# nowal/MASt3R-SLAM

Hardware: AMD Instinct MI355X
Metric: keyframe-pair GN iters/sec @512×384, 256 edges; ATE-RMSE vs ref (higher is better)
Workload: dtype f32; 1 GPU; cfg3: gauss_newton_calib op call, 256 keyframe-pair edges (512 directed), 128 keyframes, 384x512, 10 GN iters/step, delta_thresh=0; edges=256, directed_edges=512, keyframes=128, H=384, W=512, parallelism=edge-sharded x1

## Files before the change

include/m3s_backend.h:

```cpp
#ifndef M3S_BACKEND_H
#define M3S_BACKEND_H

#include <stddef.h>
#include <stdint.h>

#ifdef __cplusplus
extern "C" {
#endif

enum {
    M3S_OK = 0,
    M3S_ERR_INVALID = 1,
    M3S_ERR_HIP = 2,
    M3S_ERR_WORKSPACE = 3,
    M3S_ERR_COMM = 4,
    M3S_ERR_TIMEOUT = 5
};

const char* m3s_last_error(void);
const char* m3s_version(void);
void m3s_shutdown(void);

enum {
    M3S_CONTRACT_NVCC = 0,
// ... 4 lines not shown

int m3s_iter_proj(const float* rays, const float* pts, const float* p_init,
                  float* p_new, uint8_t* converged,
                  int64_t B, int64_t H, int64_t W, int64_t N,
                  int max_iter, float lambda_init, float cost_thresh, void* stream);
int m3s_iter_proj_ex(const float* rays, const float* pts, const float* p_init,
                     float* p_new, uint8_t* converged,
                     int64_t B, int64_t H, int64_t W, int64_t N,
                     int max_iter, float lambda_init, float cost_thresh, int contract, void* stream);

int m3s_refine_matches_f16(const uint16_t* D11, const uint16_t* D21,
                           const int64_t* p1, int64_t* p1_new,
                           int64_t B, int64_t H, int64_t W, int64_t N, int64_t F,
                           int radius, int dilation_max, void* stream);
int m3s_refine_matches_f32(const float* D11, const float* D21,
                           const int64_t* p1, int64_t* p1_new,
                           int64_t B, int64_t H, int64_t W, int64_t N, int64_t F,
                           int radius, int dilation_max, void* stream);
int m3s_refine_matches_f64(const double* D11, const double* D21,
                           const int64_t* p1, int64_t* p1_new,
                           int64_t B, int64_t H, int64_t W, int64_t N, int64_t F,
                           int radius, int dilation_max, void* stream);

size_t m3s_match_workspace_bytes(int64_t B, int64_t H, int64_t W, int64_t F);
int m3s_match_iterative_proj(const float* X11, const float* X21, const float* D11, const float* D21,
                             const int64_t* idx_init, int64_t B, int64_t H, int64_t W, int64_t F,
                             int max_iter, float lambda_init, float cost_thresh, float dist_thresh,
                             int radius, int dilation_max, int contract, int64_t* idx_out,
                             uint8_t* valid_out, void* ws, size_t ws_bytes, void* stream);



void m3s_gn_debug_flags(int* out4);
void m3s_gn_pcg_stats(int* out5);
void m3s_gn_pcg_plan(int* out5);

int m3s_gn_check(void* stream);

enum { M3S_GN_POINTS = 0, M3S_GN_RAYS = 1, M3S_GN_CALIB = 2 };

typedef struct m3s_gn_args {
    int mode;
    float* Twc;
    const float* Xs;
    const float* Cs;
    const int64_t* ii;
    const int64_t* jj;
    const int64_t* idx;
    const uint8_t* valid;
    const float* Q;
    int64_t N, HW, E_total, E_local, edge_offset;
    float sigma0;
    float sigma1;
    float C_thresh, Q_thresh;
    const float* K;
    int height, width, pixel_border;
    float z_eps;
    int max_iter;
    float delta_thresh;
    float* dx;
    void* ws;
    size_t ws_bytes;
    void* comm;
    void* stream;
    int order;
    const int64_t* idx_b;
// ... 128 lines not shown
```

mast3r-slam_amd/csrc/gn_accum.hip:

```cpp
#include <hip/hip_runtime.h>

#include <algorithm>
#include <climits>
#include <cstdint>

#include "edge_reduce.h"
#include "gn_kernels.h"
#include "sim3.h"
#include "wave_reduce.h"

#ifndef M3S_ACC_SCHED_BARRIER
#define M3S_ACC_SCHED_BARRIER 0
#endif
#ifndef M3S_ACC_DIAG
#define M3S_ACC_DIAG 0
#endif

namespace m3s {

template <typename V>
struct VMask {
    typedef bool type;
};

// ... 278 lines not shown
}

__device__ __forceinline__ void block_partial(const float* accs, float* __restrict__ out, bool coh = false) {
    __shared__ float red[kAccThreads / 64][kNaccPad];
    const int tid = threadIdx.x, lane = tid & 63, wave = tid >> 6;
    static_assert(kNaccPad == 36, "reduce-scatter is laid out for 36 values");
    float w[18], x[9];
#pragma unroll
    for (int j = 0; j < 18; j++) w[j] = halfsum32(accs[j], j + 18 < kNacc ? accs[j + 18] : 0.0f);
#pragma unroll
    for (int j = 0; j < 9; j++) x[j] = row_sum16(halfsum16(w[j], w[j + 9]));
    if ((lane & 15) == 0) {
        const int r = lane >> 4;
#pragma unroll
        for (int j = 0; j < 9; j++) red[wave][j + 9 * r] = x[j];
    }
    __syncthreads();
    if (tid < kNacc) {
        float s = red[0][tid];
#pragma unroll
        for (int w = 1; w < kAccThreads / 64; w++) s += red[w][tid];
        if (coh)
            __hip_atomic_store(out + tid, s, __ATOMIC_RELAXED, __HIP_MEMORY_SCOPE_AGENT);
        else
            out[tid] = s;
    }
}


#ifndef M3S_RC_FACTOR
#define M3S_RC_FACTOR 1
#endif

template <int MODE, bool RC = false, bool PK = true, int NP = 4>
struct AccStage {
    static_assert(NP == 4 || NP == 2, "4 or 2 points per step");
    int cd[NP], sb[NP];
    __device__ __forceinline__ void set(int4 a, int4 b) {
        cd[0] = a.x; sb[0] = a.y; cd[1] = a.z; sb[1] = a.w;
        if constexpr (NP == 4) {
            cd[2] = b.x; sb[2] = b.y; cd[3] = b.z; sb[3] = b.w;
        }
    }
    float xv[3 * NP];
    float g[NP][3];
    const float* rc_tu = nullptr;
    const float* rc_tv = nullptr;
    unsigned rc_m = 0;
    int rc_sh = 0, rc_w = 1;
    int width = 1;

    template <int M>
    __device__ __forceinline__ void load(const float* __restrict__ Xj_b, const float* __restrict__ Xi_b,
                                         const float* __restrict__ Zi_b, int k) {
        if constexpr (RC) {
            const unsigned q = (unsigned)(((uint64_t)(unsigned)k * rc_m) >> rc_sh);
            const int u = k - (int)q * rc_w;
            if constexpr (NP == 4) {
                const float4 za = *reinterpret_cast<const float4*>(Xj_b + k);
                const float4 ta = *reinterpret_cast<const float4*>(rc_tu + u);
                const float t[8] = {za.x, za.y, za.z, za.w, ta.x, ta.y, ta.z, ta.w};
#pragma unroll
                for (int i = 0; i < 8; i++) xv[i] = t[i];
            } else {
                const float2 za = *reinterpret_cast<const float2*>(Xj_b + k);
                const float2 ta = *reinterpret_cast<const float2*>(rc_tu + u);
                xv[0] = za.x; xv[1] = za.y; xv[2] = ta.x; xv[3] = ta.y;
            }
            xv[2 * NP] = rc_tv[q];
        } else if constexpr (NP == 4) {
            const float4 a = *reinterpret_cast<const float4*>(Xj_b + (int64_t)k * 3);
            const float4 b = *reinterpret_cast<const float4*>(Xj_b + (int64_t)k * 3 + 4);
            const float4 c = *reinterpret_cast<const float4*>(Xj_b + (int64_t)k * 3 + 8);
            const float t[12] = {a.x, a.y, a.z, a.w, b.x, b.y, b.z, b.w, c.x, c.y, c.z, c.w};
#pragma unroll
            for (int i = 0; i < 12; i++) xv[i] = t[i];
        } else {
            const float2 a = *reinterpret_cast<const float2*>(Xj_b + (int64_t)k * 3);
            const float2 b = *reinterpret_cast<const float2*>(Xj_b + (int64_t)k * 3 + 2);
            const float2 c = *reinterpret_cast<const float2*>(Xj_b + (int64_t)k * 3 + 4);
            const float t[6] = {a.x, a.y, b.x, b.y, c.x, c.y};
#pragma unroll
            for (int i = 0; i < 6; i++) xv[i] = t[i];
        }
        int ind[NP];
#pragma unroll
        for (int s = 0; s < NP; s++) ind[s] = (M == GN_CALIB && PK) ? uv_index(cd[s], width) : (cd[s] & 0x7fffffff);
#pragma unroll
        for (int s = 0; s < NP; s++) {
            if constexpr (M == GN_CALIB) {
                if constexpr (PK)
                    g[s][2] = Zi_b[ind[s]];
                else
                    g[s][2] = Xi_b[(int64_t)ind[s] * 3 + 2];
            } else {
                const float* xp = Xi_b + (int64_t)ind[s] * 3;
                g[s][0] = xp[0];
                g[s][1] = xp[1];
                g[s][2] = xp[2];
            }
        }
    }

    template <int M>
    __device__ __forceinline__ void compute(const RelXf& T, const AccParams& P, float* __restrict__ acc) const {
        const int* codes = cd;
        const int* sqb = sb;
        float xj[3 * NP];
        constexpr bool kFactor = RC && M == GN_CALIB && M3S_RC_FACTOR;
        float Xr[3 * NP];
        if constexpr (kFactor) {
            const float tv = xv[2 * NP];
            const float B0 = fmaf(T.m[1], tv, T.m[2]), B1 = fmaf(T.m[4], tv, T.m[5]), B2 = fmaf(T.m[7], tv, T.m[8]);
#pragma unroll
            for (int s = 0; s < NP; s++) {
                const float z = xv[s], tu = xv[NP + s];
                Xr[3 * s] = fmaf(z, fmaf(T.m[0], tu, B0), T.t[0]);
                Xr[3 * s + 1] = fmaf(z, fmaf(T.m[3], tu, B1), T.t[1]);
                Xr[3 * s + 2] = fmaf(z, fmaf(T.m[6], tu, B2), T.t[2]);
            }
        } else if constexpr (RC) {
#pragma unroll
            for (int s = 0; s < NP; s++) {
                xj[3 * s] = xv[s] * xv[NP + s];
                xj[3 * s + 1] = xv[s] * xv[2 * NP];
                xj[3 * s + 2] = xv[s];
            }
        } else {
#pragma unroll
            for (int q = 0; q < 3 * NP; q++) xj[q] = xv[q];
        }
#pragma unroll
// ... 376 lines not shown
                const int ind = match_index(ids[s], vm[s], P.HW);
                const bool ok = vm[s] && (qs[s] > P.Q_thresh) && (raw.ci_all || raw.Ci_b[ind] > P.C_thresh) &&
                                (raw.cj_all || cjs[s] > P.C_thresh);
                code[s] = pack_code(ind, ok, P);
                sqb[s] = __float_as_int(sqrt_cr(qs[s]));
            }
            a = int4{code[0], sqb[0], code[1], sqb[1]};
            raw.pk_w[kk / 2] = a;
        } else if constexpr (FIRST) {
            const uchar4 vm4 = *reinterpret_cast<const uchar4*>(raw.valid + kk);
            const longlong2 id01 = *reinterpret_cast<const longlong2*>(raw.idx + kk);
            const longlong2 id23 = *reinterpret_cast<const longlong2*>(raw.idx + kk + 2);
            const float4 q4 = *reinterpret_cast<const float4*>(raw.Q + kk);
            const float4 cj4 =
                raw.cj_all ? make_float4(0.f, 0.f, 0.f, 0.f) : *reinterpret_cast<const float4*>(raw.Cj_b + kk);
            const bool vm[4] = {vm4.x != 0, vm4.y != 0, vm4.z != 0, vm4.w != 0};
            const int64_t ids[4] = {id01.x, id01.y, id23.x, id23.y};
            const float qs[4] = {q4.x, q4.y, q4.z, q4.w};
            const float cjs[4] = {cj4.x, cj4.y, cj4.z, cj4.w};
            int code[4], sqb[4];
#pragma unroll
            for (int s = 0; s < 4; s++) {
                const int ind = match_index(ids[s], vm[s], P.HW);
                const bool ok = vm[s] && (qs[s] > P.Q_thresh) && (raw.ci_all || raw.Ci_b[ind] > P.C_thresh) &&
                                (raw.cj_all || cjs[s] > P.C_thresh);
                code[s] = pack_code(ind, ok, P);
                sqb[s] = __float_as_int(sqrt_cr(qs[s]));
            }
            a = int4{code[0], sqb[0], code[1], sqb[1]};
            b = int4{code[2], sqb[2], code[3], sqb[3]};
            raw.pk_w[kk / 2] = a;
            raw.pk_w[kk / 2 + 1] = b;
        } else {
            a = pk_b[kk / 2];
            if constexpr (NP == 4) b = pk_b[kk / 2 + 1];
        }
    };
    int4 na = int4{0, 0, 0, 0}, nb = int4{0, 0, 0, 0};
    int k = k0 + NP * threadIdx.x;
    if (k < k1) records(k, na, nb);
    for (; k < k1; k += S) {
#if M3S_ACC_DIAG == 1
        if (k == k0 + NP * (int)threadIdx.x) {
            cur.set(na, nb);
            cur.template load<MODE>(Xj_b, Xi_b, Zi_b, k);
        }
        cur.template compute<MODE>(T, P, acc);
        __builtin_amdgcn_sched_barrier(0);
        continue;
#elif M3S_ACC_DIAG == 2
        cur.set(na, nb);
        if (k + S < k1) records(k + S, na, nb);
        cur.template load<MODE>(Xj_b, Xi_b, Zi_b, k);
        if (k == k0 + NP * (int)threadIdx.x) {
            cur.template compute<MODE>(T, P, acc);
        } else {
#pragma unroll
            for (int q = 0; q < 3 * NP; q++) asm volatile("" ::"v"(cur.xv[q]));
#pragma unroll
            for (int q = 0; q < NP; q++) asm volatile("" ::"v"(cur.g[q][2]), "v"(cur.g[q][0]), "v"(cur.cd[q]), "v"(cur.sb[q]));
        }
        continue;
#endif
        cur.set(na, nb);
        if (k + S < k1) records(k + S, na, nb);
        cur.template load<MODE>(Xj_b, Xi_b, Zi_b, k);
        cur.template compute<MODE>(T, P, acc);
    }
}


#ifndef M3S_ACC_WAVES
#define M3S_ACC_WAVES 1
#endif
#ifndef M3S_ACC_WAVES_RAYS
#define M3S_ACC_WAVES_RAYS M3S_ACC_WAVES
#endif
template <int MODE, bool FIRST>
constexpr int acc_waves() {
    return (MODE == GN_RAYS && !FIRST) ? M3S_ACC_WAVES_RAYS : M3S_ACC_WAVES;
}
struct FirstSrc {
    EdgeSrc es;
    const float* Cs;
    const int* cok;
    int4* pack_w;
};

template <int MODE, bool COMPACT, bool RCOK = false, bool FIRST = false>
__global__ __launch_bounds__(kAccThreads) __attribute__((amdgpu_waves_per_eu(acc_waves<MODE, FIRST>())))
void gn_accum_packed_kernel(
    const float* __restrict__ Twc, const float* __restrict__ Xs, const float* __restrict__ Zs,
    const int* __restrict__ ii_loc, const int* __restrict__ jj_loc, const int4* __restrict__ pack,
    AccParams P, const int4* __restrict__ sched, float* __restrict__ partials,
    const int* __restrict__ flags, const float* __restrict__ px, const int* __restrict__ pcnt,
    int* __restrict__ ecnt, double* __restrict__ edgeblk, FirstSrc fs) {
    const int4 tk = sched[blockIdx.x];
    if (flags[kFlagDone]) return;
    const int e = tk.x, c = tk.y, ix = tk.z, jx = tk.w;
    const RelXf T = rel_xf(rel_sim3(load_sim3(Twc + (int64_t)ix * 8), load_sim3(Twc + (int64_t)jx * 8)));

    const int HW = P.HW;
    const int64_t ebase = (int64_t)e * HW;
    const float* __restrict__ Xi_b = Xs + (int64_t)ix * HW * 3;
    const float* __restrict__ Zi_b = MODE == GN_CALIB ? inv_depths(Zs, P) + (int64_t)ix * HW : nullptr;
    const float* __restrict__ Xj_b = Xs + (int64_t)jx * HW * 3;
    const int4* __restrict__ pk_b = pack + ebase / 2;
    const int k0 = c * P.chunk;
    const int k1 = min(k0 + P.chunk, HW);

    float acc[kNacc];
#pragma unroll
    for (int q = 0; q < kNacc; q++) acc[q] = 0.0f;
    if constexpr (COMPACT) {
        const int64_t cb = ((int64_t)e * P.nchunks + c) * P.chunk;
        accum_steps<MODE, false, acc_np<MODE>()>(px + cb * 3, Xi_b, Zi_b, pack + cb / 2, 0, pcnt[(int64_t)e * P.nchunks + c], T, P,
                                 Zs, acc);
    } else if constexpr (FIRST) {
        RawSrc raw;
        fs.es.at(e, HW, raw.idx, raw.valid, raw.Q);
        raw.Ci_b = fs.Cs + (int64_t)ix * HW;
        raw.Cj_b = fs.Cs + (int64_t)jx * HW;
        raw.pk_w = fs.pack_w + ebase / 2;
        raw.ci_all = fs.cok != nullptr && fs.cok[ix] != 0;
        raw.cj_all = fs.cok != nullptr && fs.cok[jx] != 0;
        if (RCOK && flags[kFlagNotRay] == 0 && (P.width & 3) == 0)
            accum_steps<MODE, true, 4, true>(Zs + (int64_t)jx * HW, Xi_b, Zi_b, pk_b, k0, k1, T, P, Zs, acc, raw);
        else
            accum_steps<MODE, false, acc_np<MODE>(), true>(Xj_b, Xi_b, Zi_b, pk_b, k0, k1, T, P, Zs, acc, raw);
    } else if (RCOK && MODE == GN_CALIB && flags[kFlagNotRay] == 0 && (P.width & 3) == 0)
        accum_steps<MODE, true, acc_np<MODE>()>(Zs + (int64_t)jx * HW, Xi_b, Zi_b, pk_b, k0, k1, T, P, Zs, acc);
    else
        accum_steps<MODE, false, acc_np<MODE>()>(Xj_b, Xi_b, Zi_b, pk_b, k0, k1, T, P, Zs, acc);
    block_partial(acc, partials + ((int64_t)e * P.nchunks + c) * kNaccPad, ecnt != nullptr);
    if (ecnt != nullptr) {
        __shared__ int s_last;
        asm volatile("s_waitcnt vmcnt(0)" ::: "memory");
        __syncthreads();
        if (threadIdx.x == 0)
            s_last = __hip_atomic_fetch_add(ecnt + e, 1, __ATOMIC_RELAXED, __HIP_MEMORY_SCOPE_AGENT) == P.nchunks - 1;
        __syncthreads();
        if (s_last) {
            edge_reduce_body<true>(partials, P.nchunks, Twc, ii_loc, edgeblk, e);
            if (threadIdx.x == 0) __hip_atomic_store(ecnt + e, 0, __ATOMIC_RELAXED, __HIP_MEMORY_SCOPE_AGENT);
        }
    }
}

hipError_t launch_accum(int mode, bool vec, dim3 grid, hipStream_t st, const float* Twc,
                        const float* Xs, const float* Cs, const int* ii_loc, const int* jj_loc,
                        const EdgeSrc& es, const AccParams& P, const int4* sched, float* partials,
                        const int* flags) {
#define M3S_ACC(MODE, V)                                                                    \
    hipLaunchKernelGGL((gn_accum_kernel<MODE, V>), grid, dim3(kAccThreads), 0, st, Twc, Xs, \
                       Cs, ii_loc, jj_loc, es, P, sched, partials, flags)
    if (mode == GN_RAYS) {
        if (vec) M3S_ACC(GN_RAYS, true); else M3S_ACC(GN_RAYS, false);
    } else if (mode == GN_CALIB) {
        if (vec) M3S_ACC(GN_CALIB, true); else M3S_ACC(GN_CALIB, false);
    } else {
        if (vec) M3S_ACC(GN_POINTS, true); else M3S_ACC(GN_POINTS, false);
    }
#undef M3S_ACC
    return hipGetLastError();
}

hipError_t launch_pack_pre(hipStream_t st, const float* Xs, int64_t N, const float* Cs, const AccParams& P, int* cok,
                           float* Zs, int* flags, const float* K) {
    if (cok != nullptr && N > 0) {
        const int bx = (int)std::max<int64_t>(1, std::min<int64_t>((P.HW + 1023) / 1024, 8192 / std::max<int64_t>(N, 1)));
        hipLaunchKernelGGL(gn_cpass_kernel, dim3(bx, (unsigned)N), dim3(256), 0, st, Cs, P, cok, flags);
    }
    if (Zs) {
        const int64_t total = N * (int64_t)P.HW;
        const int bx = (int)std::max<int64_t>(std::min<int64_t>((P.HW + 255) / 256,
                                                                std::max<int64_t>(8192 / std::max<int64_t>(N, 1), 2)),
                                              (std::max(P.width, P.height) + 255) / 256);
        hipLaunchKernelGGL(gn_depth_kernel, dim3(bx, (unsigned)N), dim3(256), 0, st, Xs, total, Zs, P, flags, K);
    }
    return hipGetLastError();
}

hipError_t launch_pack(int mode, hipStream_t st, int E_local, const float* Xs, int64_t N, const float* Cs,
                       const int* ii_loc, const int* jj_loc, const EdgeSrc& es, const AccParams& P, int* cok,
                       int4* pack, float* px, int* pcnt, const int* flags, bool skip_pack) {
    if (E_local > 0 && px) {
        const dim3 grid((unsigned)P.nchunks, (unsigned)E_local);
        int2* pk = reinterpret_cast<int2*>(pack);
        if (mode == GN_RAYS)
            hipLaunchKernelGGL(gn_pack_compact_kernel<GN_RAYS>, grid, dim3(kAccThreads), 0, st, Xs, Cs, ii_loc,
                               jj_loc, es, P, pk, px, pcnt, flags);
        else if (mode == GN_CALIB)
            hipLaunchKernelGGL(gn_pack_compact_kernel<GN_CALIB>, grid, dim3(kAccThreads), 0, st, Xs, Cs, ii_loc,
                               jj_loc, es, P, pk, px, pcnt, flags);
        else
            hipLaunchKernelGGL(gn_pack_compact_kernel<GN_POINTS>, grid, dim3(kAccThreads), 0, st, Xs, Cs, ii_loc,
                               jj_loc, es, P, pk, px, pcnt, flags);
    } else if (E_local > 0) {
        const dim3 grid((unsigned)((P.HW / 4 + kAccThreads - 1) / kAccThreads), (unsigned)E_local);
        if (!skip_pack)
            hipLaunchKernelGGL(gn_pack_kernel, grid, dim3(kAccThreads), 0, st, Cs, ii_loc, jj_loc, es,
                               P, cok, pack, flags);
    }
    return hipGetLastError();
}

hipError_t launch_accum_packed(int mode, dim3 grid, hipStream_t st, const float* Twc,
                               const float* Xs, const float* Zs, const int* ii_loc,
                               const int* jj_loc, const int4* pack, const AccParams& P,
                               const int4* sched, float* partials, const int* flags, const float* px,
                               const int* pcnt, int* ecnt, double* edgeblk, const EdgeSrc* first_es,
                               const float* Cs, const int* cok) {
    if (first_es != nullptr) {
        if (px != nullptr) return hipErrorInvalidValue;
        const FirstSrc fs{*first_es, Cs, cok, const_cast<int4*>(pack)};
        if (mode == GN_RAYS)
            hipLaunchKernelGGL((gn_accum_packed_kernel<GN_RAYS, false, false, true>), grid, dim3(kAccThreads), 0, st,
                               Twc, Xs, Zs, ii_loc, jj_loc, pack, P, sched, partials, flags, px, pcnt, ecnt,
                               edgeblk, fs);
        else if (mode == GN_POINTS)
            hipLaunchKernelGGL((gn_accum_packed_kernel<GN_POINTS, false, false, true>), grid, dim3(kAccThreads), 0, st,
                               Twc, Xs, Zs, ii_loc, jj_loc, pack, P, sched, partials, flags, px, pcnt, ecnt,
                               edgeblk, fs);
        else if (P.raycheck)
            hipLaunchKernelGGL((gn_accum_packed_kernel<GN_CALIB, false, true, true>), grid, dim3(kAccThreads), 0, st,
                               Twc, Xs, Zs, ii_loc, jj_loc, pack, P, sched, partials, flags, px, pcnt, ecnt,
                               edgeblk, fs);
        else
            hipLaunchKernelGGL((gn_accum_packed_kernel<GN_CALIB, false, false, true>), grid, dim3(kAccThreads), 0, st,
                               Twc, Xs, Zs, ii_loc, jj_loc, pack, P, sched, partials, flags, px, pcnt, ecnt,
                               edgeblk, fs);
        return hipGetLastError();
    }
    const FirstSrc fs0{};
#define M3S_ACCP(MODE, CP, RC)                                                                       \
    hipLaunchKernelGGL((gn_accum_packed_kernel<MODE, CP, RC>), grid, dim3(kAccThreads), 0, st, Twc, Xs, Zs, \
                       ii_loc, jj_loc, pack, P, sched, partials, flags, px, pcnt, ecnt, edgeblk, fs0)
#define M3S_ACCP2(MODE, CP) M3S_ACCP(MODE, CP, false)
    const bool cp = px != nullptr;
    if (mode == GN_RAYS) {
        if (cp) M3S_ACCP2(GN_RAYS, true); else M3S_ACCP2(GN_RAYS, false);
    } else if (mode == GN_CALIB) {
        if (cp) M3S_ACCP2(GN_CALIB, true);
        else if (P.raycheck) M3S_ACCP(GN_CALIB, false, true);
        else M3S_ACCP2(GN_CALIB, false);
    } else {
        if (cp) M3S_ACCP2(GN_POINTS, true); else M3S_ACCP2(GN_POINTS, false);
    }
#undef M3S_ACCP2
#undef M3S_ACCP
    return hipGetLastError();
}

}
```

mast3r-slam_amd/csrc/gn_driver.hip:

```cpp
#include <hip/hip_runtime.h>

#include <algorithm>
#include <chrono>
#include <cstdlib>
#include <cstdarg>
#include <cstdio>
#include <cstring>
#include <functional>
#include <map>
#include <mutex>
#include <set>
#include <string>
#include <utility>
#include <vector>

#include "../../include/m3s_backend.h"
#include "gn_kernels.h"
#include "m3s_common.h"
#include "m3s_comm.h"
#include "sparse_plan.h"

namespace m3s {

namespace {
// ... 6 lines not shown
    std::vector<hipEvent_t> pool;
    std::vector<hipEvent_t> marks;
    hipEvent_t get() {
        if (pool.empty()) {
            static const bool sysfence = env_int("M3S_PROF_SYSFENCE", 0) != 0;
            hipEvent_t e;
            if (sysfence || hipEventCreateWithFlags(&e, hipEventDisableSystemFence) != hipSuccess) {
                (void)hipGetLastError();
                if (hipEventCreate(&e) != hipSuccess) return nullptr;
            }
            return e;
        }
        hipEvent_t e = pool.back();
        pool.pop_back();
        return e;
    }
    bool accum_only = false;
    std::vector<char> first;
    void mark(hipStream_t st, bool accum = false, bool first_pack = false) {
        if (!on || (accum_only && !accum)) return;
        hipEvent_t e = get();
        if (e && hipEventRecord(e, st) == hipSuccess) {
            marks.push_back(e);
            if (accum_only && marks.size() % 2 == 0) first.push_back(first_pack);
        }
    }
};
Prof g_prof;
std::vector<double> g_prof_launch_ms;
std::vector<double> g_prof_solve_ms;
}

int g_dbg_flags[4] = {0, 0, 0, 0};
int g_dbg_pcg[5] = {0, 0, 0, 0, 0};
int g_dbg_pcg_plan[5] = {0, 0, 0, 0, 0};

void set_error(const char* fmt, ...) {
    char buf[1024];
    va_list ap;
    va_start(ap, fmt);
    vsnprintf(buf, sizeof(buf), fmt, ap);
    va_end(ap);
    g_err = buf;
}

const char* get_error() { return g_err.c_str(); }

namespace {
struct HostResources {
    std::mutex mu;
    std::vector<std::pair<void*, void (*)(void*)>> items;
    bool shut = false;
};
HostResources& host_resources() {
    static HostResources* r = new HostResources;
    return *r;
}
}

void register_host_resource(void* obj, void (*release)(void*)) {
    HostResources& r = host_resources();
    std::lock_guard<std::mutex> lk(r.mu);
    r.items.emplace_back(obj, release);
}

namespace {
// ... 580 lines not shown
                "gauss_newton_calib: K / image size required");
    M3S_REQUIRE(a.Twc && a.Xs && a.Cs && a.dx, "gauss_newton: null pointer");
    if (a.E_total > 0) M3S_REQUIRE(a.ii && a.jj, "gauss_newton: null ii/jj");
    if (a.E_local > 0) M3S_REQUIRE(a.idx && a.valid && a.Q, "gauss_newton: null edge data");
    if (a.idx_b || a.valid_b || a.Q_b) {
        M3S_REQUIRE(a.idx_b && a.valid_b && a.Q_b, "gauss_newton: incomplete second edge half");
        M3S_REQUIRE(a.E_a >= 0 && a.E_a <= a.E_local, "gauss_newton: bad edge split E_a = %lld",
                    (long long)a.E_a);
    }
    const size_t need = make_layout(a.mode, a.N, a.HW, a.E_total, a.E_local).total;
    M3S_REQUIRE(a.ws != nullptr && a.ws_bytes >= need,
                "gauss_newton: workspace too small (%zu < %zu bytes)", a.ws_bytes, need);
    return M3S_OK;
}

Plan& tls_plan() {
    static thread_local Plan p;
    return p;
}
SparsePlan& tls_sparse_plan() {
    static thread_local SparsePlan sp;
    return sp;
}

struct Ctx {
    bool need_slotmap = false;
    bool packed = false;
    bool compact = false;
    bool ref_order = false;
    bool pack_issued = false;
    bool acc_enqueued = false;
    bool gathered = false;
    bool first_pack = false;
    RefParams R;
    Layout L;
    Plan& plan = tls_plan();
    SparsePlan& sp = tls_sparse_plan();
    AccParams P;
    EdgeSrc es{};
    bool vec;
    char* ws;
    hipStream_t st = nullptr;
    char* dyn = nullptr;
    size_t o_dense = 0, o_linv = 0, o_slot = 0;
    double* eall = nullptr;
    double* eblk() const {
        return eall ? eall + (size_t)plan.grank * plan.gchunk * kEdgeBlk : at<double>(L.edgeblk);
    }
    const double* eblk_all() const { return eall ? eall : at<double>(L.edgeblk); }
    int chol_epoch = 0;
    int pcg_launches = 0;
    bool inv_pending = false;
    hipEvent_t inv_done = nullptr;
    bool may_timeout = false;
    template <typename T>
    T* at(size_t off) const { return reinterpret_cast<T*>(ws + off); }
    template <typename T>
    T* dyn_at(size_t off) const { return reinterpret_cast<T*>(dyn + off); }
    int alloc_dense(int npad, int npose) {
        size_t off = 0;
        auto take = [&](size_t bytes) {
            size_t o = off;
            off = align_up(off + std::max<size_t>(bytes, 8), 256);
            return o;
        };
        o_dense = take(sizeof(double) * (size_t)(npad + kCholTile) * npad);
// ... 44 lines not shown
    const auto s0 = std::chrono::steady_clock::now();
    const Layout& L = c.L;
    AccParams& P = c.P;
    P.s0_inv = 1.0f / a.sigma0;
    P.s1_inv = (a.mode == M3S_GN_POINTS) ? 0.0f : 1.0f / a.sigma1;
    P.C_thresh = a.C_thresh;
    P.Q_thresh = a.Q_thresh;
    P.pb_lo = (float)a.pixel_border;
    P.pb_hi_u = (float)(a.width - 1 - a.pixel_border);
    P.pb_hi_v = (float)(a.height - 1 - a.pixel_border);
    P.z_eps = a.z_eps;
    P.width = a.width > 0 ? a.width : 1;
    P.height = a.height;
    {
        int l = 0;
        while ((1LL << l) < P.width) l++;
        const unsigned long long num = 1ULL << (31 + l);
        P.div_m = (unsigned)((num + (unsigned long long)P.width - 1) / (unsigned long long)P.width);
        P.div_sh = 31 + l;
    }
    P.HW = (int)a.HW;
    P.chunk = chunk_points(a.HW, L.nchunks);
    P.nchunks = L.nchunks;
    P.nkf = (int)a.N;
    auto al16 = [](const void* ptr) { return ((uintptr_t)ptr & 15) == 0; };
    const bool two = a.idx_b != nullptr;
    c.es.idx[0] = a.idx;
    c.es.valid[0] = a.valid;
    c.es.Q[0] = a.Q;
    c.es.idx[1] = two ? a.idx_b : a.idx;
    c.es.valid[1] = two ? a.valid_b : a.valid;
    c.es.Q[1] = two ? a.Q_b : a.Q;
    c.es.E_a = two ? (int)a.E_a : (int)a.E_local;
    c.vec = (a.HW % 4 == 0) && al16(a.Xs) && al16(a.Cs) && al16(a.idx) && al16(a.valid) &&
            al16(a.Q) && (!two || (al16(a.idx_b) && al16(a.valid_b) && al16(a.Q_b)));
    const int pack_mode = env_int("M3S_GN_PACK", 1);
    c.packed = c.vec && a.E_local > 0 && (pack_mode == 2 || (pack_mode == 1 && a.max_iter >= 3));
    c.compact = c.packed && env_int("M3S_GN_COMPACT", 0) != 0;
    if (a.mode == M3S_GN_CALIB && (a.width >= 65536 || a.height >= 32768)) c.packed = c.compact = false;
    P.pack_uv = c.packed && a.mode == M3S_GN_CALIB;
    P.raycheck = c.packed && !c.compact && a.mode == M3S_GN_CALIB && env_int("M3S_GN_RAYCHECK", 1) != 0;

    c.ref_order = gn_order(a) == M3S_GN_ORDER_REFERENCE;
    if (c.ref_order) {
        c.packed = false;
        RefParams& R = c.R;
        R.s0_inv = (float)(1.0 / (double)a.sigma0);
        R.s1_inv = (a.mode == M3S_GN_POINTS) ? 0.0f : (float)(1.0 / (double)a.sigma1);
        R.C_thresh = a.C_thresh;
        R.Q_thresh = a.Q_thresh;
        R.z_eps = a.z_eps;
        R.width = a.width > 0 ? a.width : 1;
        R.height = a.height;
        R.pixel_border = a.pixel_border;
        R.HW = a.HW;
        R.variant = env_int("M3S_GN_REF_VARIANT", 0);
        R.contract = a.contract;
    }
    int* dflags = c.at<int>(L.flags);
    int* dcok = c.at<int>(L.cok);
    auto pre_pass = [&]() -> int {
        M3S_HIP_CHECK(launch_gn_init(c.st, dflags, P.raycheck ? 0 : 1, dcok, a.N));
        if (c.packed)
            M3S_HIP_CHECK(launch_pack_pre(c.st, a.Xs, a.N, a.Cs, P, !c.compact ? dcok : nullptr,
                                          a.mode == M3S_GN_CALIB ? c.at<float>(L.zs) : nullptr, dflags,
                                          a.mode == M3S_GN_CALIB ? a.K : nullptr));
        return M3S_OK;
// ... 91 lines not shown
                                       c.R, c.at<float>(L.edgeblk), flags));
        g_prof.mark(c.st, true);
        SparsePlan& sp = c.sp;
        double* sys = sp.dptr<double>(sp.o_sys);
        M3S_HIP_CHECK(launch_assemble_ref(c.st, c.at<float>(L.edgeblk), c.at<int>(L.blk_ptr),
                                          c.at<int>(L.blk_ref), c.at<int>(L.grad_ptr),
                                          c.at<int>(L.grad_ent), c.plan.nblk, sp.nblocks, npose_r,
                                          sp.bpad, sys, flags));
        if (a.comm) {
            const size_t count = (size_t)sp.bpad + (size_t)c.plan.nblk * 49;
            int rc = comm_allreduce_sum_f64(a.comm, sys, count, c.st);
            if (rc) return rc;
        }
        return M3S_OK;
    }
    if (!c.acc_enqueued) {
        int rc = enqueue_accumulate(a, c);
        if (rc) return rc;
    }
    c.acc_enqueued = false;
    return enqueue_assembly(a, c);
}

int enqueue_accumulate(const m3s_gn_args& a, Ctx& c) {
    const Layout& L = c.L;
    int* flags = c.at<int>(L.flags);
    if (a.E_local > 0) {
        g_prof.mark(c.st, true);
        const dim3 grid((unsigned)(L.nchunks * a.E_local));
        const bool fuse_reduce = env_int("M3S_GN_FUSE_REDUCE", 1) != 0;
        const bool fused = c.packed && fuse_reduce;
        const bool was_first = c.packed && c.first_pack;
        if (c.packed) {
            M3S_HIP_CHECK(launch_accum_packed(a.mode, grid, c.st, a.Twc, a.Xs, c.at<float>(L.zs),
                                              c.at<int>(L.ii_loc), c.at<int>(L.jj_loc),
                                              c.at<int4>(L.pack), c.P, c.at<int4>(L.sched),
                                              c.at<float>(L.partials), flags,
                                              c.compact ? c.at<float>(L.packx) : nullptr,
                                              c.at<int>(L.pcnt), fused ? c.at<int>(L.ecnt) : nullptr,
                                              c.eblk(), c.first_pack ? &c.es : nullptr,
                                              a.Cs, c.at<int>(L.cok)));
            c.first_pack = false;
        } else
            M3S_HIP_CHECK(launch_accum(a.mode, c.vec, grid, c.st, a.Twc, a.Xs, a.Cs,
                                       c.at<int>(L.ii_loc), c.at<int>(L.jj_loc), c.es, c.P,
                                       c.at<int4>(L.sched), c.at<float>(L.partials),
                                       flags));
        g_prof.mark(c.st, true, was_first);
        if (!fused)
            M3S_HIP_CHECK(launch_edge_reduce((int)a.E_local, c.st, c.at<float>(L.partials), L.nchunks,
                                             a.Twc, c.at<int>(L.ii_loc), c.eblk(), flags));
    }
    return M3S_OK;
}

int enqueue_assembly(const m3s_gn_args& a, Ctx& c) {
    const Layout& L = c.L;
    int* flags = c.at<int>(L.flags);
    const int npose = (int)(a.N - 1);
    if (c.plan.gather && !c.gathered) {
        int rc = comm_allgather_f64(a.comm, c.eall, (size_t)c.plan.gchunk * kEdgeBlk, c.st);
        if (rc) return rc;
    }
    c.gathered = false;
    const bool reduce = a.comm && !c.plan.gather;
    if (c.sp.enabled) {
        SparsePlan& sp = c.sp;
        double* sys = sp.dptr<double>(sp.o_sys);
        M3S_HIP_CHECK(launch_assemble(c.st, c.eblk_all(), c.at<int>(L.blk_ptr),
                                      c.at<int>(L.blk_ent), c.at<int>(L.grad_ptr),
                                      c.at<int>(L.grad_ent), c.plan.nblk, sp.nblocks, npose, sp.bpad,
                                      sys, flags));
        if (reduce) {
            const size_t count = (size_t)sp.bpad + (size_t)c.plan.nblk * 49;
// ... 552 lines not shown
        char* h = sg.tmo.get(64);
        M3S_REQUIRE(h != nullptr, "gauss_newton: pinned host allocation failed");
        float* save = c.at<float>(L.twc_save);
        const int n8 = (int)(8 * a.N);
        if (a.comm) {
            double* dv = c.at<double>(L.x);
            M3S_HIP_CHECK(launch_flag_export(c.st, flags + kFlagTimeout, dv, 1));
            rc = comm_allreduce_sum_f64(a.comm, dv, 1, c.st);
            if (rc) return rc;
            M3S_HIP_CHECK(launch_twc_restore_on_flag(c.st, a.Twc, save, n8, dv, 1, sg.tmo.dev));
            if (!sg.tmo.dev) M3S_HIP_CHECK(hipMemcpyAsync(h, dv, sizeof(double), hipMemcpyDeviceToHost, c.st));
            sg.tmo_armed = 2;
        } else {
            M3S_HIP_CHECK(launch_twc_restore_on_flag(c.st, a.Twc, save, n8, flags + kFlagTimeout, 0, sg.tmo.dev));
            if (!sg.tmo.dev)
                M3S_HIP_CHECK(hipMemcpyAsync(h, flags + kFlagTimeout, sizeof(int), hipMemcpyDeviceToHost, c.st));
            sg.tmo_armed = 1;
        }
        M3S_HIP_CHECK(sg.tmo.mark(c.st));
        static const bool sync_report = env_int("M3S_GN_TIMEOUT_SYNC", 0) != 0;
        if (sync_report) {
            rc = take_deferred_timeout("");
            if (rc) return rc;
        }
    }
    if (const int dbg = env_int("M3S_GN_DEBUG_FLAGS", 0)) {
        int hf[kNumFlags];
        M3S_HIP_CHECK(hipMemcpyAsync(hf, flags, sizeof(hf), hipMemcpyDeviceToHost, c.st));
        M3S_HIP_CHECK(hipStreamSynchronize(c.st));
        g_dbg_flags[0] = hf[kFlagDone];
        g_dbg_flags[1] = hf[kFlagFail];
        g_dbg_flags[2] = c.packed ? 1 : 0;
        g_dbg_flags[3] = (c.packed && c.P.raycheck && hf[kFlagNotRay] == 0) ? 1 : 0;
        g_dbg_pcg[0] = hf[kFlagPcgRuns];
        g_dbg_pcg[1] = hf[kFlagPcgSteps];
        g_dbg_pcg[2] = hf[kFlagPcgFall];
        g_dbg_pcg[3] = c.sp.pcg ? 1 : 0;
        g_dbg_pcg[4] = c.sp.pcg ? c.sp.pcg_from : 0;
        g_dbg_pcg_plan[0] = c.sp.pcg ? c.sp.pcg_R : 0;
        g_dbg_pcg_plan[1] = c.sp.pcg ? c.sp.pcg_nwg : 0;
        g_dbg_pcg_plan[2] = c.sp.pcg && c.sp.pcg_onex ? 1 : 0;
        g_dbg_pcg_plan[3] = c.sp.pcg ? c.sp.pcg_lag : 0;
        g_dbg_pcg_plan[4] = c.sp.pcg ? c.sp.pcg_nitem : 0;
        if (dbg != 2)
            fprintf(stderr, "gn flags: done %d fail %d not_ray %d timeout %d packed %d pcg runs %d steps %d fallbacks %d\n",
                    hf[kFlagDone], hf[kFlagFail], hf[kFlagNotRay], hf[kFlagTimeout], (int)c.packed,
                    hf[kFlagPcgRuns], hf[kFlagPcgSteps], hf[kFlagPcgFall]);
    }
    return M3S_OK;
}

}
}

using namespace m3s;

extern "C" const char* m3s_last_error(void) { return m3s::get_error(); }

extern "C" int m3s_gn_check(void* stream) {
    const hipError_t e = hipStreamSynchronize(static_cast<hipStream_t>(stream));
    if (e != hipSuccess) {
        set_error("gn_check: %s", hipGetErrorString(e));
        return M3S_ERR_HIP;
    }
    return m3s::take_deferred_timeout("");
}

extern "C" void m3s_gn_debug_flags(int* out4) {
    for (int k = 0; k < 4; k++) out4[k] = m3s::g_dbg_flags[k];
}

extern "C" void m3s_gn_pcg_stats(int* out5) {
    for (int k = 0; k < 5; k++) out5[k] = m3s::g_dbg_pcg[k];
}

extern "C" void m3s_gn_pcg_plan(int* out5) {
    for (int k = 0; k < 5; k++) out5[k] = m3s::g_dbg_pcg_plan[k];
}

extern "C" const char* m3s_version(void) { return "m3s 0.1.0 gfx950"; }

extern "C" void m3s_shutdown(void) {
    HostResources& r = host_resources();
    std::lock_guard<std::mutex> lk(r.mu);
    if (r.shut) return;
    r.shut = true;
    for (auto& it : r.items) it.second(it.first);
    r.items.clear();
}

namespace {
__attribute__((constructor)) void m3s_register_shutdown() { std::atexit(m3s_shutdown); }
}

extern "C" size_t m3s_gn_workspace_bytes(int mode, int64_t N, int64_t HW, int64_t E_total,
                                         int64_t E_local) {
    if (N < 1 || HW < 1 || E_total < 0 || E_local < 0) return 0;
    return make_layout(mode, N, HW, E_total, E_local).total;
}

extern "C" int m3s_gn_plan_info(const int64_t* ii, const int64_t* jj, int64_t E, int64_t N, int32_t* info,
                                int32_t* order, int32_t* round_ptr, int32_t round_cap) {
// ... 261 lines not shown
```

mast3r-slam_amd/csrc/gn_kernels.h:

```cpp
#pragma once

#include <hip/hip_runtime.h>

#include <cstdint>

namespace m3s {

enum { GN_POINTS = 0, GN_RAYS = 1, GN_CALIB = 2 };

#ifndef M3S_ACC_THREADS
#define M3S_ACC_THREADS 256
#endif
constexpr int kAccThreads = M3S_ACC_THREADS;
constexpr int kNacc = 35;
constexpr int kNaccPad = 36;
constexpr int kEdgeBlk = 36;
constexpr int kCholTile = 64;

constexpr int kFlagDone = 0;
constexpr int kFlagFail = 1;
constexpr int kFlagNotRay = 2;
constexpr int kFlagTimeout = 3;
constexpr int kFlagBarCount = 4;
constexpr int kFlagBarGen = 5;
constexpr int kFlagSkipSolve = 6;
constexpr int kFlagPcgRuns = 7;
constexpr int kFlagPcgSteps = 8;
constexpr int kFlagPcgFall = 9;
constexpr int kFlagPcgAbort = 10;
constexpr int kNumFlags = 16;
__device__ __forceinline__ bool solve_skipped(const int* flags) {
    return (flags[kFlagDone] | flags[kFlagSkipSolve]) != 0;
}

struct EdgeSrc {
    const int64_t* idx[2];
    const uint8_t* valid[2];
    const float* Q[2];
    int E_a;
    __device__ __forceinline__ void at(int e, int64_t HW, const int64_t*& i, const uint8_t*& v,
                                       const float*& q) const {
        const int h = e >= E_a;
        const int64_t off = (int64_t)(h ? e - E_a : e) * HW;
        i = idx[h] + off;
        v = valid[h] + off;
        q = Q[h] + off;
    }
};

__host__ __device__ constexpr int sym_idx(int a, int b) {
    return a * 7 - a * (a - 1) / 2 + (b - a);
}

struct AccParams {
    float s0_inv, s1_inv;
    float C_thresh, Q_thresh;
    float fx, fy, cx, cy;
    float pb_lo, pb_hi_u, pb_hi_v;
    float z_eps;
    unsigned div_m;
    int div_sh;
    int width, height;
// ... 13 lines not shown
    float fx, fy, cx, cy;
    float z_eps;
    int width, height, pixel_border;
    int64_t HW;
    int variant;
    int contract;
};
constexpr int kRefVarLogRatio = 1;
constexpr int kRefVarRcp = 2;
constexpr int kRefVarHuberMin = 4;
hipError_t launch_accum_ref(int mode, int E_local, hipStream_t st, const float* Twc, const float* Xs,
                            const float* Cs, const int* ii_loc, const int* jj_loc, const EdgeSrc& es,
                            const RefParams& P, float* out, const int* flags);
hipError_t launch_assemble_ref(hipStream_t st, const float* ref, const int* blk_ptr, const int* blk_ref,
                               const int* grad_ptr, const int* grad_ent, int nblk, int nblocks,
                               int npose, int bpad, double* out, const int* flags);

hipError_t launch_accum(int mode, bool vec, dim3 grid, hipStream_t st, const float* Twc,
                        const float* Xs, const float* Cs, const int* ii_loc, const int* jj_loc,
                        const EdgeSrc& es, const AccParams& P, const int4* sched, float* partials,
                        const int* flags);
hipError_t launch_pack(int mode, hipStream_t st, int E_local, const float* Xs, int64_t N, const float* Cs,
                       const int* ii_loc, const int* jj_loc, const EdgeSrc& es, const AccParams& P, int* cok,
                       int4* pack, float* px, int* pcnt, const int* flags, bool skip_pack = false);
hipError_t launch_pack_pre(hipStream_t st, const float* Xs, int64_t N, const float* Cs, const AccParams& P, int* cok,
                           float* Zs, int* flags, const float* K);
hipError_t launch_gn_init(hipStream_t st, int* flags, int not_ray, int* cok, int64_t n);
hipError_t launch_accum_packed(int mode, dim3 grid, hipStream_t st, const float* Twc,
                               const float* Xs, const float* Zs, const int* ii_loc,
                               const int* jj_loc, const int4* pack, const AccParams& P,
                               const int4* sched, float* partials, const int* flags, const float* px,
                               const int* pcnt, int* ecnt = nullptr, double* edgeblk = nullptr,
                               const EdgeSrc* first_es = nullptr, const float* Cs = nullptr,
                               const int* cok = nullptr);
hipError_t launch_edge_reduce(int E_local, hipStream_t st, const float* partials, int nchunks,
                              const float* Twc, const int* ii_loc, double* edgeblk,
                              const int* flags);
hipError_t launch_compact(hipStream_t st, const double* edgeblk, const int* blk_ptr,
                          const int* blk_ent, const int* grad_ptr, const int* grad_ent, int nblk,
                          int npose, double* compact, const int* flags);
hipError_t launch_assemble(hipStream_t st, const double* edgeblk, const int* blk_ptr,
                           const int* blk_ent, const int* grad_ptr, const int* grad_ent, int nblk,
                           int nblocks, int npose, int bpad, double* out, const int* flags);
hipError_t launch_solve(hipStream_t st, const double* compact, const int* slotmap, int nblk,
                        int npose, int n, int npad, double* Hd, double* Linv, double* x,
                        int* flags, int epoch);
constexpr int kMaxNpad = 8192;
size_t chol_ready_bytes(int npad);
inline size_t chol_linv_bytes(int npad) {
    return sizeof(double) * (size_t)npad * kCholTile + chol_ready_bytes(npad);
}
inline int* chol_ready_ptr(double* Linv, int npad) {
    return reinterpret_cast<int*>(Linv + (size_t)npad * kCholTile);
}
struct DfScatter {
    const int* tail;
    int ntail;
    double* xpose;
};
hipError_t launch_chol_dataflow(hipStream_t st, int npad, double* Hd, double* Linv, int* ready,
                                int epoch, int* flags, double* x = nullptr, const DfScatter* g = nullptr);
hipError_t launch_dense_factor_solve(hipStream_t st, int npad, double* Hd, double* Linv,
                                     double* x, int* flags, int epoch, const DfScatter* g = nullptr);
hipError_t launch_sp_tail_scatter(hipStream_t st, const double* xd, const int* tail, int ntail, double* x,
                                  const int* flags);
constexpr int kSpInline = 9;
constexpr int kSpRec = 4 + 4 * kSpInline;
// ... 120 lines not shown
```

Before: 570,600 keyframe-pair GN iters/s.

## Serpentine accum block order across GN iterations and use 32-bit offset loads

On every odd accumulation launch, blocks are remapped so each residue class mod 8 walks its schedule in reverse. The aim is for the edges processed last in one iteration to be processed first in the next, while their data may still be in L2/MALL. The change also replaces 64-bit pointer arithmetic in the inner loads with 32-bit byte offsets, gated on HW < 2^28, and restructures the record-prefetch loop into a ping-pong of two register sets. It adds a debug counter (one atomic per launch) and an exported query for it.

New measurement: 574,200 keyframe-pair GN iters/s, median of 6. No clear change (+0.6%).

```diff
diff --git a/include/m3s_backend.h b/include/m3s_backend.h
--- a/include/m3s_backend.h
+++ b/include/m3s_backend.h
@@ -60,6 +60,7 @@
 
 
 void m3s_gn_debug_flags(int* out4);
+void m3s_gn_accum_order(int* out2);
 void m3s_gn_pcg_stats(int* out5);
 void m3s_gn_pcg_plan(int* out5);
 
diff --git a/mast3r-slam_amd/csrc/gn_accum.hip b/mast3r-slam_amd/csrc/gn_accum.hip
--- a/mast3r-slam_amd/csrc/gn_accum.hip
+++ b/mast3r-slam_amd/csrc/gn_accum.hip
@@ -334,6 +334,11 @@
 #define M3S_RC_FACTOR 1
 #endif
 
+template <typename T, typename B>
+__device__ __forceinline__ T ld_off(const B* base, unsigned elem, unsigned elem_bytes = sizeof(B)) {
+    return *reinterpret_cast<const T*>(reinterpret_cast<const char*>(base) + elem * elem_bytes);
+}
+
 template <int MODE, bool RC = false, bool PK = true, int NP = 4>
 struct AccStage {
     static_assert(NP == 4 || NP == 2, "4 or 2 points per step");
@@ -359,28 +364,28 @@
             const unsigned q = (unsigned)(((uint64_t)(unsigned)k * rc_m) >> rc_sh);
             const int u = k - (int)q * rc_w;
             if constexpr (NP == 4) {
-                const float4 za = *reinterpret_cast<const float4*>(Xj_b + k);
-                const float4 ta = *reinterpret_cast<const float4*>(rc_tu + u);
+                const float4 za = ld_off<float4>(Xj_b, k);
+                const float4 ta = ld_off<float4>(rc_tu, u);
                 const float t[8] = {za.x, za.y, za.z, za.w, ta.x, ta.y, ta.z, ta.w};
 #pragma unroll
                 for (int i = 0; i < 8; i++) xv[i] = t[i];
             } else {
-                const float2 za = *reinterpret_cast<const float2*>(Xj_b + k);
-                const float2 ta = *reinterpret_cast<const float2*>(rc_tu + u);
+                const float2 za = ld_off<float2>(Xj_b, k);
+                const float2 ta = ld_off<float2>(rc_tu, u);
                 xv[0] = za.x; xv[1] = za.y; xv[2] = ta.x; xv[3] = ta.y;
             }
-            xv[2 * NP] = rc_tv[q];
+            xv[2 * NP] = ld_off<float>(rc_tv, q);
         } else if constexpr (NP == 4) {
-            const float4 a = *reinterpret_cast<const float4*>(Xj_b + (int64_t)k * 3);
-            const float4 b = *reinterpret_cast<const float4*>(Xj_b + (int64_t)k * 3 + 4);
-            const float4 c = *reinterpret_cast<const float4*>(Xj_b + (int64_t)k * 3 + 8);
+            const float4 a = ld_off<float4>(Xj_b, k, 12);
+            const float4 b = ld_off<float4>(Xj_b + 4, k, 12);
+            const float4 c = ld_off<float4>(Xj_b + 8, k, 12);
             const float t[12] = {a.x, a.y, a.z, a.w, b.x, b.y, b.z, b.w, c.x, c.y, c.z, c.w};
 #pragma unroll
             for (int i = 0; i < 12; i++) xv[i] = t[i];
         } else {
-            const float2 a = *reinterpret_cast<const float2*>(Xj_b + (int64_t)k * 3);
-            const float2 b = *reinterpret_cast<const float2*>(Xj_b + (int64_t)k * 3 + 2);
-            const float2 c = *reinterpret_cast<const float2*>(Xj_b + (int64_t)k * 3 + 4);
+            const float2 a = ld_off<float2>(Xj_b, k, 12);
+            const float2 b = ld_off<float2>(Xj_b + 2, k, 12);
+            const float2 c = ld_off<float2>(Xj_b + 4, k, 12);
             const float t[6] = {a.x, a.y, b.x, b.y, c.x, c.y};
 #pragma unroll
             for (int i = 0; i < 6; i++) xv[i] = t[i];
@@ -392,14 +397,13 @@
         for (int s = 0; s < NP; s++) {
             if constexpr (M == GN_CALIB) {
                 if constexpr (PK)
-                    g[s][2] = Zi_b[ind[s]];
+                    g[s][2] = ld_off<float>(Zi_b, ind[s]);
                 else
-                    g[s][2] = Xi_b[(int64_t)ind[s] * 3 + 2];
+                    g[s][2] = ld_off<float>(Xi_b + 2, ind[s], 12);
             } else {
-                const float* xp = Xi_b + (int64_t)ind[s] * 3;
-                g[s][0] = xp[0];
-                g[s][1] = xp[1];
-                g[s][2] = xp[2];
+                g[s][0] = ld_off<float>(Xi_b, ind[s], 12);
+                g[s][1] = ld_off<float>(Xi_b + 1, ind[s], 12);
+                g[s][2] = ld_off<float>(Xi_b + 2, ind[s], 12);
             }
         }
     }
@@ -842,27 +846,24 @@
             raw.pk_w[kk / 2] = a;
             raw.pk_w[kk / 2 + 1] = b;
         } else {
-            a = pk_b[kk / 2];
-            if constexpr (NP == 4) b = pk_b[kk / 2 + 1];
+            a = ld_off<int4>(pk_b, kk, 8);
+            if constexpr (NP == 4) b = ld_off<int4>(pk_b + 1, kk, 8);
         }
     };
-    int4 na = int4{0, 0, 0, 0}, nb = int4{0, 0, 0, 0};
-    int k = k0 + NP * threadIdx.x;
-    if (k < k1) records(k, na, nb);
-    for (; k < k1; k += S) {
+    const int kfirst = k0 + NP * (int)threadIdx.x;
+    auto step = [&](int kk, const int4& a, const int4& b, int4& na, int4& nb) {
 #if M3S_ACC_DIAG == 1
-        if (k == k0 + NP * (int)threadIdx.x) {
-            cur.set(na, nb);
-            cur.template load<MODE>(Xj_b, Xi_b, Zi_b, k);
+        if (kk == kfirst) {
+            cur.set(a, b);
+            cur.template load<MODE>(Xj_b, Xi_b, Zi_b, kk);
         }
         cur.template compute<MODE>(T, P, acc);
         __builtin_amdgcn_sched_barrier(0);
-        continue;
 #elif M3S_ACC_DIAG == 2
-        cur.set(na, nb);
-        if (k + S < k1) records(k + S, na, nb);
-        cur.template load<MODE>(Xj_b, Xi_b, Zi_b, k);
-        if (k == k0 + NP * (int)threadIdx.x) {
+        cur.set(a, b);
+        cur.template load<MODE>(Xj_b, Xi_b, Zi_b, kk);
+        if (kk + S < k1) records(kk + S, na, nb);
+        if (kk == kfirst) {
             cur.template compute<MODE>(T, P, acc);
         } else {
 #pragma unroll
@@ -870,12 +871,22 @@
 #pragma unroll
             for (int q = 0; q < NP; q++) asm volatile("" ::"v"(cur.g[q][2]), "v"(cur.g[q][0]), "v"(cur.cd[q]), "v"(cur.sb[q]));
         }
-        continue;
-#endif
-        cur.set(na, nb);
-        if (k + S < k1) records(k + S, na, nb);
-        cur.template load<MODE>(Xj_b, Xi_b, Zi_b, k);
+#else
+        cur.set(a, b);
+        cur.template load<MODE>(Xj_b, Xi_b, Zi_b, kk);
+        if (kk + S < k1) records(kk + S, na, nb);
         cur.template compute<MODE>(T, P, acc);
+#endif
+    };
+    int4 a0 = int4{0, 0, 0, 0}, b0 = int4{0, 0, 0, 0}, a1 = int4{0, 0, 0, 0}, b1 = int4{0, 0, 0, 0};
+    int k = kfirst;
+    if (k < k1) records(k, a0, b0);
+    while (k < k1) {
+        step(k, a0, b0, a1, b1);
+        k += S;
+        if (k >= k1) break;
+        step(k, a1, b1, a0, b0);
+        k += S;
     }
 }
 
@@ -896,6 +907,13 @@
     const int* cok;
     int4* pack_w;
 };
+
+__device__ __forceinline__ unsigned accum_task(unsigned b, unsigned n, int rev) {
+    if (!rev) return b;
+    const unsigned r = b & 7u;
+    const unsigned cnt = (n - r + 7u) >> 3;
+    return r + 8u * (cnt - 1u - (b >> 3));
+}
 
 template <int MODE, bool COMPACT, bool RCOK = false, bool FIRST = false>
 __global__ __launch_bounds__(kAccThreads) __attribute__((amdgpu_waves_per_eu(acc_waves<MODE, FIRST>())))
@@ -904,8 +922,8 @@
     const int* __restrict__ ii_loc, const int* __restrict__ jj_loc, const int4* __restrict__ pack,
     AccParams P, const int4* __restrict__ sched, float* __restrict__ partials,
     const int* __restrict__ flags, const float* __restrict__ px, const int* __restrict__ pcnt,
-    int* __restrict__ ecnt, double* __restrict__ edgeblk, FirstSrc fs) {
-    const int4 tk = sched[blockIdx.x];
+    int* __restrict__ ecnt, double* __restrict__ edgeblk, FirstSrc fs, int rev) {
+    const int4 tk = sched[accum_task(blockIdx.x, gridDim.x, rev)];
     if (flags[kFlagDone]) return;
     const int e = tk.x, c = tk.y, ix = tk.z, jx = tk.w;
     const RelXf T = rel_xf(rel_sim3(load_sim3(Twc + (int64_t)ix * 8), load_sim3(Twc + (int64_t)jx * 8)));
@@ -955,6 +973,8 @@
             if (threadIdx.x == 0) __hip_atomic_store(ecnt + e, 0, __ATOMIC_RELAXED, __HIP_MEMORY_SCOPE_AGENT);
         }
     }
+    if (rev && blockIdx.x == 0 && threadIdx.x == 0)
+        __hip_atomic_fetch_add(const_cast<int*>(flags) + kFlagAccRev, 1, __ATOMIC_RELAXED, __HIP_MEMORY_SCOPE_AGENT);
 }
 
 hipError_t launch_accum(int mode, bool vec, dim3 grid, hipStream_t st, const float* Twc,
@@ -1020,32 +1040,33 @@
                                const int* jj_loc, const int4* pack, const AccParams& P,
                                const int4* sched, float* partials, const int* flags, const float* px,
                                const int* pcnt, int* ecnt, double* edgeblk, const EdgeSrc* first_es,
-                               const float* Cs, const int* cok) {
+                               const float* Cs, const int* cok, bool reverse) {
+    const int rev = reverse ? 1 : 0;
     if (first_es != nullptr) {
         if (px != nullptr) return hipErrorInvalidValue;
         const FirstSrc fs{*first_es, Cs, cok, const_cast<int4*>(pack)};
         if (mode == GN_RAYS)
             hipLaunchKernelGGL((gn_accum_packed_kernel<GN_RAYS, false, false, true>), grid, dim3(kAccThreads), 0, st,
                                Twc, Xs, Zs, ii_loc, jj_loc, pack, P, sched, partials, flags, px, pcnt, ecnt,
-                               edgeblk, fs);
+                               edgeblk, fs, rev);
         else if (mode == GN_POINTS)
             hipLaunchKernelGGL((gn_accum_packed_kernel<GN_POINTS, false, false, true>), grid, dim3(kAccThreads), 0, st,
                                Twc, Xs, Zs, ii_loc, jj_loc, pack, P, sched, partials, flags, px, pcnt, ecnt,
-                               edgeblk, fs);
+                               edgeblk, fs, rev);
         else if (P.raycheck)
             hipLaunchKernelGGL((gn_accum_packed_kernel<GN_CALIB, false, true, true>), grid, dim3(kAccThreads), 0, st,
                                Twc, Xs, Zs, ii_loc, jj_loc, pack, P, sched, partials, flags, px, pcnt, ecnt,
-                               edgeblk, fs);
+                               edgeblk, fs, rev);
         else
             hipLaunchKernelGGL((gn_accum_packed_kernel<GN_CALIB, false, false, true>), grid, dim3(kAccThreads), 0, st,
                                Twc, Xs, Zs, ii_loc, jj_loc, pack, P, sched, partials, flags, px, pcnt, ecnt,
-                               edgeblk, fs);
+                               edgeblk, fs, rev);
         return hipGetLastError();
     }
     const FirstSrc fs0{};
 #define M3S_ACCP(MODE, CP, RC)                                                                       \
     hipLaunchKernelGGL((gn_accum_packed_kernel<MODE, CP, RC>), grid, dim3(kAccThreads), 0, st, Twc, Xs, Zs, \
-                       ii_loc, jj_loc, pack, P, sched, partials, flags, px, pcnt, ecnt, edgeblk, fs0)
+                       ii_loc, jj_loc, pack, P, sched, partials, flags, px, pcnt, ecnt, edgeblk, fs0, rev)
 #define M3S_ACCP2(MODE, CP) M3S_ACCP(MODE, CP, false)
     const bool cp = px != nullptr;
     if (mode == GN_RAYS) {
diff --git a/mast3r-slam_amd/csrc/gn_driver.hip b/mast3r-slam_amd/csrc/gn_driver.hip
--- a/mast3r-slam_amd/csrc/gn_driver.hip
+++ b/mast3r-slam_amd/csrc/gn_driver.hip
@@ -62,6 +62,7 @@
 }
 
 int g_dbg_flags[4] = {0, 0, 0, 0};
+int g_dbg_acc[2] = {0, 0};
 int g_dbg_pcg[5] = {0, 0, 0, 0, 0};
 int g_dbg_pcg_plan[5] = {0, 0, 0, 0, 0};
 
@@ -708,6 +709,7 @@
     bool acc_enqueued = false;
     bool gathered = false;
     bool first_pack = false;
+    int acc_launches = 0;
     RefParams R;
     Layout L;
     Plan& plan = tls_plan();
@@ -818,7 +820,8 @@
     c.es.valid[1] = two ? a.valid_b : a.valid;
     c.es.Q[1] = two ? a.Q_b : a.Q;
     c.es.E_a = two ? (int)a.E_a : (int)a.E_local;
-    c.vec = (a.HW % 4 == 0) && al16(a.Xs) && al16(a.Cs) && al16(a.idx) && al16(a.valid) &&
+    c.vec = (a.HW % 4 == 0) && a.HW < ((int64_t)1 << 28) && al16(a.Xs) && al16(a.Cs) && al16(a.idx) &&
+            al16(a.valid) &&
             al16(a.Q) && (!two || (al16(a.idx_b) && al16(a.valid_b) && al16(a.Q_b)));
     const int pack_mode = env_int("M3S_GN_PACK", 1);
     c.packed = c.vec && a.E_local > 0 && (pack_mode == 2 || (pack_mode == 1 && a.max_iter >= 3));
@@ -976,6 +979,8 @@
         const bool fused = c.packed && fuse_reduce;
         const bool was_first = c.packed && c.first_pack;
         if (c.packed) {
+            const bool reverse = env_int("M3S_ACC_SERPENTINE", 1) != 0 && (c.acc_launches & 1) != 0;
+            c.acc_launches++;
             M3S_HIP_CHECK(launch_accum_packed(a.mode, grid, c.st, a.Twc, a.Xs, c.at<float>(L.zs),
                                               c.at<int>(L.ii_loc), c.at<int>(L.jj_loc),
                                               c.at<int4>(L.pack), c.P, c.at<int4>(L.sched),
@@ -983,7 +988,7 @@
                                               c.compact ? c.at<float>(L.packx) : nullptr,
                                               c.at<int>(L.pcnt), fused ? c.at<int>(L.ecnt) : nullptr,
                                               c.eblk(), c.first_pack ? &c.es : nullptr,
-                                              a.Cs, c.at<int>(L.cok)));
+                                              a.Cs, c.at<int>(L.cok), reverse));
             c.first_pack = false;
         } else
             M3S_HIP_CHECK(launch_accum(a.mode, c.vec, grid, c.st, a.Twc, a.Xs, a.Cs,
@@ -1602,6 +1607,8 @@
         g_dbg_flags[1] = hf[kFlagFail];
         g_dbg_flags[2] = c.packed ? 1 : 0;
         g_dbg_flags[3] = (c.packed && c.P.raycheck && hf[kFlagNotRay] == 0) ? 1 : 0;
+        g_dbg_acc[0] = c.acc_launches;
+        g_dbg_acc[1] = hf[kFlagAccRev];
         g_dbg_pcg[0] = hf[kFlagPcgRuns];
         g_dbg_pcg[1] = hf[kFlagPcgSteps];
         g_dbg_pcg[2] = hf[kFlagPcgFall];
@@ -1638,6 +1645,10 @@
 
 extern "C" void m3s_gn_debug_flags(int* out4) {
     for (int k = 0; k < 4; k++) out4[k] = m3s::g_dbg_flags[k];
+}
+
+extern "C" void m3s_gn_accum_order(int* out2) {
+    for (int k = 0; k < 2; k++) out2[k] = m3s::g_dbg_acc[k];
 }
 
 extern "C" void m3s_gn_pcg_stats(int* out5) {
diff --git a/mast3r-slam_amd/csrc/gn_kernels.h b/mast3r-slam_amd/csrc/gn_kernels.h
--- a/mast3r-slam_amd/csrc/gn_kernels.h
+++ b/mast3r-slam_amd/csrc/gn_kernels.h
@@ -28,6 +28,7 @@
 constexpr int kFlagPcgSteps = 8;
 constexpr int kFlagPcgFall = 9;
 constexpr int kFlagPcgAbort = 10;
+constexpr int kFlagAccRev = 11;
 constexpr int kNumFlags = 16;
 __device__ __forceinline__ bool solve_skipped(const int* flags) {
     return (flags[kFlagDone] | flags[kFlagSkipSolve]) != 0;
@@ -107,7 +108,7 @@
                                const int4* sched, float* partials, const int* flags, const float* px,
                                const int* pcnt, int* ecnt = nullptr, double* edgeblk = nullptr,
                                const EdgeSrc* first_es = nullptr, const float* Cs = nullptr,
-                               const int* cok = nullptr);
+                               const int* cok = nullptr, bool reverse = false);
 hipError_t launch_edge_reduce(int E_local, hipStream_t st, const float* partials, int nchunks,
                               const float* Twc, const int* ii_loc, double* edgeblk,
                               const int* flags);
```
